# PacificBiosciences/minorseq

Hardware: NVIDIA B200
Metric: aligned CCS reads/sec pileup+call+phase (higher is better)
Workload: dtype u32 counts / f64 p-values

## Files before the change

### minorseq_b200/csrc/call.cu

```cuda
#include <algorithm>
#include <cstring>
#include <vector>
#include "fisher_core.h"
#include "handle.h"

namespace ms {

struct CallPos {
    int32_t gene, codon_index, col, ref_codon;
    uint32_t ntests;
};

struct CallConst {
    double P[4];
    double alpha, min_perc, max_perc;
};

__global__ void call_kernel(const uint32_t* __restrict__ codon, const CallPos* __restrict__ pos, int32_t npos,
                            CallConst cc, ms_variant* __restrict__ out, unsigned long long* __restrict__ nout,
                            unsigned long long cap) {
    const int warp = (blockIdx.x * blockDim.x + threadIdx.x) >> 5, lane = threadIdx.x & 31;
    if (warp >= npos) return;
    const CallPos ps = pos[warp];
    const uint32_t* h = codon + static_cast<size_t>(ps.col) * 64;
    const uint32_t k0 = h[lane], k1 = h[lane + 32];
    uint32_t n = k0 + k1;
#pragma unroll
    for (int o = 16; o > 0; o >>= 1) n += __shfl_xor_sync(0xffffffffu, n, o);
    if (n == 0) return;
    int ref = ps.ref_codon;
    if (ref < 0) {
        uint32_t bc = k0, bi = lane;
        if (k1 > bc) { bc = k1; bi = lane + 32; }
#pragma unroll
        for (int o = 16; o > 0; o >>= 1) {
            const uint32_t oc = __shfl_xor_sync(0xffffffffu, bc, o), oi = __shfl_xor_sync(0xffffffffu, bi, o);
            if (oc > bc || (oc == bc && oi < bi)) { bc = oc; bi = oi; }
        }
        ref = static_cast<int>(bi);
    }
#pragma unroll
    for (int half = 0; half < 2; ++half) {
        const int c = lane + 32 * half;
        const uint32_t k = half ? k1 : k0;
        if (c == ref || k == 0) continue;
        int nm = 0;
#pragma unroll
        for (int i = 0; i < 3; ++i) nm += (((ref >> (2 * i)) & 3) != ((c >> (2 * i)) & 3)) ? 1 : 0;
        const double ex = ceil(static_cast<double>(n) * cc.P[nm]);
        const uint32_t e = ex >= static_cast<double>(n) ? n : static_cast<uint32_t>(ex);
        if (k <= e && 0.5 * static_cast<double>(ps.ntests) >= cc.alpha) continue;
        const double p = fisher_greater(k, n - k, e, n - e, 1.000001 * cc.alpha / static_cast<double>(ps.ntests));
        if (!(p * static_cast<double>(ps.ntests) < cc.alpha)) continue;
        const double perc = 100.0 * static_cast<double>(k) / static_cast<double>(n);
        if (cc.min_perc >= 0.0 && !(perc > cc.min_perc)) continue;
        if (cc.max_perc >= 0.0 && !(perc < cc.max_perc)) continue;
        const unsigned long long slot = atomicAdd(nout, 1ULL);
        if (slot < cap) {
            ms_variant v;
            v.gene = ps.gene; v.codon_index = ps.codon_index; v.col = ps.col; v.ref_codon = ref; v.codon = c;
            v.count = k; v.coverage = n; v.expected = e; v.ntests = ps.ntests; v.pvalue = p;
            out[slot] = v;
        }
    }
}

static int base_code(char ch) {
    switch (ch) {
    case 'A': case 'a': return 0;
    case 'C': case 'c': return 1;
    case 'G': case 'g': return 2;
    case 'T': case 't': return 3;
    default: return -1;
    }
}

}

extern "C" {

void ms_call_params_default(ms_call_params* p) {
    if (!p) return;
    p->substitution_rate = 5e-4; p->deletion_rate = 3e-3; p->alpha = 0.01;
    p->min_perc = -1.0; p->max_perc = -1.0; p->region_begin = 0; p->region_end = 0;
}

// ... 52 lines not shown
    ms_variant* d_out = reinterpret_cast<ms_variant*>(base + 64);
    ms::CallPos* d_pos = reinterpret_cast<ms::CallPos*>(base + 64 + dev_cap * sizeof(ms_variant));
    constexpr size_t kQuick = 1024;
    const size_t stage_need = std::max(npos * sizeof(ms::CallPos), 64 + kQuick * sizeof(ms_variant));
    if (stage_need > h->call_stage_cap) {
        if (h->call_stage) cudaFreeHost(h->call_stage);
        h->call_stage = nullptr; h->call_stage_cap = 0;
        MS_CUDA(h, cudaMallocHost(&h->call_stage, stage_need + 4096));
        h->call_stage_cap = stage_need + 4096;
    }
    const size_t pos_bytes = npos * sizeof(ms::CallPos);
    const bool same_pos = h->call_pos_cache.size() == pos_bytes && memcmp(h->call_pos_cache.data(), pos.data(), pos_bytes) == 0;
    MS_CUDA(h, cudaMemsetAsync(d_n, 0, 8, h->stream));
    if (!same_pos) {
        memcpy(h->call_stage, pos.data(), pos_bytes);
        MS_CUDA(h, cudaMemcpyAsync(d_pos, h->call_stage, pos_bytes, cudaMemcpyHostToDevice, h->stream));
        MS_CUDA(h, cudaStreamSynchronize(h->stream));
        h->call_pos_cache.assign(reinterpret_cast<const uint8_t*>(pos.data()), reinterpret_cast<const uint8_t*>(pos.data()) + pos_bytes);
    }
    ms::CallConst cc;
    ms::codon_error_table(prm->substitution_rate, prm->deletion_rate, cc.P);
    cc.alpha = prm->alpha; cc.min_perc = prm->min_perc; cc.max_perc = prm->max_perc;
    const int threads = 128;
    const int blocks = static_cast<int>((npos * 32 + threads - 1) / threads);
    ms::call_kernel<<<blocks, threads, 0, h->stream>>>(h->d_counts + static_cast<size_t>(L) * 8, d_pos,
                                                       static_cast<int32_t>(npos), cc, d_out, d_n, dev_cap);
    h->launches++;
    MS_CUDA(h, cudaGetLastError());
    const size_t quick = std::min(kQuick, dev_cap);
    MS_CUDA(h, cudaMemcpyAsync(h->call_stage, base, 64 + quick * sizeof(ms_variant), cudaMemcpyDeviceToHost, h->stream));
    if (d_calls) *d_calls = d_out;
    if (d_ncalls) *d_ncalls = d_n;
    if (calls_cap) *calls_cap = static_cast<int64_t>(dev_cap);
    return MS_OK;
}

int ms_call_collect(ms_handle* h, bool synced, ms_variant* out, int64_t cap, int64_t* n) {
    if (!h || !n || (cap > 0 && !out)) return MS_ERR_ARG;
    *n = 0;
    if (h->call_npos == 0) return MS_OK;
    MS_CUDA(h, cudaSetDevice(h->device));
    if (!synced) MS_CUDA(h, cudaStreamSynchronize(h->stream));
    constexpr size_t kQuick = 1024;
    const size_t dev_cap = h->call_npos * 63;
    const size_t quick = std::min(kQuick, dev_cap);
    uint8_t* base = static_cast<uint8_t*>(h->d_call_buf);
    const ms_variant* d_out = reinterpret_cast<const ms_variant*>(base + 64);
// ... 31 lines not shown
```

### minorseq_b200/csrc/handle.h

```cpp
#pragma once
#include <cuda_runtime.h>
#include <stdint.h>
#include <string>
#include <vector>
#include "../../include/minorseq_b200.h"
#include <nvtx3/nvToolsExt.h>

struct MsRange {
    explicit MsRange(const char* name) { nvtxRangePushA(name); }
    ~MsRange() { nvtxRangePop(); }
    MsRange(const MsRange&) = delete;
    MsRange& operator=(const MsRange&) = delete;
};

struct DevBuf {
    void* p = nullptr;
    size_t cap = 0;
    cudaError_t ensure(size_t bytes) {
        if (bytes <= cap && p) return cudaSuccess;
        if (p) { cudaError_t e = cudaFree(p); p = nullptr; cap = 0; if (e != cudaSuccess) return e; }
        const size_t want = bytes + bytes / 4 + 256;
        cudaError_t e = cudaMalloc(&p, want);
        if (e == cudaSuccess) cap = want;
        return e;
// ... 44 lines not shown
    bool have_base = false;

    uint32_t* d_upload = nullptr;
    size_t upload_cap = 0;
    DevBuf b_rowstage[2];

    void* d_call_buf = nullptr;
    size_t call_cap = 0;
    void* call_stage = nullptr;
    size_t call_stage_cap = 0;
    std::vector<uint8_t> call_pos_cache;
    size_t call_npos = 0;

    int32_t V = 0, vwords = 0;
    int64_t phase_cap = 0, phase_n = 0;
    int32_t nblocklist = 0;
    int32_t phase_nrec = 0;
    bool phase_ordered = true;
    bool phase_partial_all = false;
    int64_t tab_size = 0, tab_size_max = 0, tab_hint = 0;
    int64_t gcap_hint = 0;
    bool table_valid = false;
    int table_attempt = 0;
    DevBuf b_plan;
    void* plan_stage = nullptr;
    uint32_t* counts_stage = nullptr; size_t counts_stage_words = 0;
    DevBuf b_var, b_blocklist, b_bits, b_flags, b_slot, b_tab_key, b_tab_cnt, b_tab_rep, b_ctr, b_groups, b_gather, b_rank, b_hap,
        b_pat, b_cooc, b_bits_t;
    DevBuf b_gslot, b_mt_key, b_mt_cnt, b_mt_rep, b_mslot, b_mindex, b_m_cnt, b_m_pat, b_m_rank, b_ord, b_keys, b_out, b_tc_tiles;
    DevBuf b_nw_seq, b_nw_hrow, b_nw_hcol, b_nw_dir;
    int32_t tc_tiles_V = -1;
    int cooc_variant = 0;
    bool linkage = false;
    bool link_ready = false;
    bool gram_valid = false;
    std::vector<int32_t> link_col;
    DevBuf b_mbits, b_link_gram, b_link_col, b_link_sig, b_link_rows, b_link_out;
    std::vector<uint32_t> groups_cnt, groups_pat;
    uint64_t groups_marg[4] = {0, 0, 0, 0};
    bool groups_valid = false;
    void* h_stage = nullptr;
    size_t h_stage_cap = 0;

    void* comm = nullptr;
    int world = 1, rank = 0;

// ... 21 lines not shown
```

### minorseq_b200/csrc/phase.cu

```cuda
#include <algorithm>
#include <cstring>
#include <numeric>
#include <vector>
#include "phase_internal.cuh"

namespace ms {

constexpr uint32_t kHdrFirst = 1u << 24, kHdrPacked = 1u << 25;

constexpr int kPhaseWarps = 8;
constexpr int kPhaseChunkMax = 16;

template <bool kClean>
__global__ void __launch_bounds__(kPhaseWarps * 32, 4) phase_bits_kernel(
    const uint4* __restrict__ packed, int64_t R, int32_t nblk, const int32_t* __restrict__ blocklist, int32_t NB, int32_t chunk, int32_t dbuf,
    const uint32_t* __restrict__ stream, int32_t nwords, int32_t vwords, int32_t ordered, int32_t partial_all,
    uint32_t* __restrict__ bits, uint8_t* __restrict__ flags, unsigned long long* __restrict__ ctr, const PhasePlan* __restrict__ plan,
    uint32_t* __restrict__ mbits) {
    extern __shared__ __align__(16) uint4 stage_sm[];
    if (plan) {
        if (plan->fallback) return;
        NB = plan->NB; nwords = plan->nwords; partial_all = plan->partial_all; ordered = 1;
    }
    const int warp = threadIdx.x >> 5, lane = threadIdx.x & 31;
    uint4* sm = stage_sm + static_cast<size_t>(warp) * (dbuf ? 2 : 1) * (chunk + 1) * 32 + lane;
    const int64_t nwarps = static_cast<int64_t>(gridDim.x) * kPhaseWarps;
    unsigned long long c_dam = 0, c_gap = 0, c_het = 0, c_par = 0;
    for (int64_t base = (static_cast<int64_t>(blockIdx.x) * kPhaseWarps + warp) * 32; base < R; base += nwarps * 32) {
        const int64_t r = base + lane;
        const bool live = r < R;
        const uint4* tile = packed + static_cast<size_t>(r >> 3) * nblk * 8;
        const uint32_t pos = static_cast<uint32_t>(r & 7);
        uint32_t fg = 0, fh = 0, fp = partial_all ? 1u : 0u;
        uint32_t word = 0, widx = 0xffffffffu;
        uint32_t mword = 0;
        uint32_t* myrow = bits + static_cast<size_t>(r) * vwords;
        uint32_t* mrow = kClean ? mbits + static_cast<size_t>(r) * vwords : nullptr;
        auto flush = [&]() {
            if (ordered) myrow[widx] = word;
            else if (word) myrow[widx] |= word;
            if constexpr (kClean) {
                if (ordered) mrow[widx] = mword;
                else if (mword) mrow[widx] |= mword;
            }
        };
// ... 89 lines not shown
                    if constexpr (kClean) mword |= __funnelshift_l(0u, __funnelshift_r(clean, 0u, w) & 1u, v);
                }
                p += nv;
            }
            __syncwarp();
            if (!dbuf && c0 + chunk < NB) stage_chunk(c0 + chunk, sm0);
        }
        if (live) {
            if (ordered && vwords == 1) {
                myrow[0] = word;
                if constexpr (kClean) mrow[0] = mword;
            } else if (widx != 0xffffffffu) {
                flush();
            }
            const uint32_t f = (fg ? MS_FLAG_GAP : 0) | (fh ? MS_FLAG_HET : 0) | (fp ? MS_FLAG_PARTIAL : 0);
            flags[r] = static_cast<uint8_t>(f);
            if (f) {
                ++c_dam;
                if (f & MS_FLAG_GAP) ++c_gap;
                if (f & MS_FLAG_HET) ++c_het;
                if (f & MS_FLAG_PARTIAL) ++c_par;
            }
        }
    }
#pragma unroll
    for (int o = 16; o > 0; o >>= 1) {
        c_dam += __shfl_xor_sync(0xffffffffu, c_dam, o);
        c_gap += __shfl_xor_sync(0xffffffffu, c_gap, o);
        c_het += __shfl_xor_sync(0xffffffffu, c_het, o);
        c_par += __shfl_xor_sync(0xffffffffu, c_par, o);
    }
    if (lane == 0 && c_dam) {
        atomicAdd(ctr + 0, c_dam);
        atomicAdd(ctr + 1, c_gap);
        atomicAdd(ctr + 2, c_het);
        atomicAdd(ctr + 3, c_par);
    }
}

constexpr int kPlanSlotWords = kPlanMaxLayers * 5 + kPlanMaxKeys;

__device__ __forceinline__ void rank_distinct(const int32_t* vals, int n, int lane, int32_t* first, int (&rank)[2]) {
    for (int e = 0; e < 2; ++e) {
        const int i = lane + 32 * e;
        int f = 0;
        if (i < n && vals[i] != 0x7fffffff) {
            f = 1;
            for (int j = 0; j < i; ++j) f &= vals[j] != vals[i];
        }
        first[i] = f;
    }
    __syncwarp();
    for (int e = 0; e < 2; ++e) {
        const int i = lane + 32 * e;
        int r = 0;
        if (i < n)
            for (int j = 0; j < n; ++j) r += (first[j] && vals[j] < vals[i]) ? 1 : 0;
        rank[e] = r;
    }
// ... 97 lines not shown
    }
    __syncwarp();
    if (s_fail) return;
    int total = 0;
    for (int e = 0; e < 2; ++e) {
        const int sl = lane + 32 * e;
        int off = 0;
        for (int t = 0; t < sl; ++t) off += s_nw[t];
        for (int k = 0; k < s_nw[sl]; ++k) stream[off + k] = s_words[sl][k];
        if (sl < NB) blocklist[sl] = s_blk[sl];
    }
    for (int t = 0; t < kPlanMaxBlocks; ++t) total += s_nw[t];
    if (lane < V) { plan->key_col[lane] = s_kc[lane]; plan->key_codon[lane] = s_kk[lane]; }
    __syncwarp();
    if (lane == 0) {
        plan->V = V; plan->NB = NB; plan->nwords = total; plan->partial_all = partial;
        __threadfence();
        plan->fallback = 0;
    }
}

__global__ void __launch_bounds__(256) phase_clear_kernel(unsigned long long* __restrict__ tab_key, uint32_t* __restrict__ tab_cnt,
                                                          long long* __restrict__ tab_rep, int64_t tab_size, unsigned long long* __restrict__ ctr,
                                                          unsigned long long last_resort) {
    const int64_t stride = static_cast<int64_t>(gridDim.x) * blockDim.x;
    for (int64_t i = static_cast<int64_t>(blockIdx.x) * blockDim.x + threadIdx.x; i < tab_size; i += stride) {
        tab_key[i] = 0ULL;
        tab_cnt[i] = 0u;
        tab_rep[i] = 0x7f7f7f7f7f7f7f7fLL;
    }
    if (blockIdx.x == 0 && threadIdx.x == 0) { ctr[4] = 0ULL; ctr[6] = 0ULL; ctr[7] = last_resort; }
}

__global__ void phase_insert_kernel(const uint32_t* __restrict__ bits, const uint8_t* __restrict__ flags, int64_t R,
                                    int32_t vwords, uint64_t seed, unsigned long long* tab_key, uint32_t* tab_cnt,
                                    long long* tab_rep, int64_t mask, int32_t* __restrict__ slot, unsigned long long* overflow) {
    const int64_t r = static_cast<int64_t>(blockIdx.x) * blockDim.x + threadIdx.x;
    const int lane = threadIdx.x & 31;
    const bool valid = r < R && flags[r] == 0;
    if (r < R && !valid) slot[r] = -1;
    if (__any_sync(0xffffffffu, *reinterpret_cast<volatile unsigned long long*>(overflow) != 0ULL)) {
        if (r < R) slot[r] = -1;
        return;
    }
    const uint32_t vmask = __ballot_sync(0xffffffffu, valid);
    if (!valid) return;
    const uint64_t key = pattern_hash(bits + static_cast<size_t>(r) * vwords, vwords, seed);
    const uint32_t peers = __match_any_sync(vmask, static_cast<unsigned long long>(key));
    const int leader = __ffs(peers) - 1;
    int64_t idx = -1;
    if (lane == leader) {
        int64_t probe = static_cast<int64_t>(key) & mask;
        for (int step = 0; step < 256; ++step) {
            const unsigned long long prev = atomicCAS(tab_key + probe, 0ULL, static_cast<unsigned long long>(key));
            if (prev == 0ULL || prev == key) { idx = probe; break; }
            probe = (probe + 1) & mask;
        }
        if (idx >= 0) {
            atomicAdd(tab_cnt + idx, static_cast<uint32_t>(__popc(peers)));
            atomicMin(tab_rep + idx, static_cast<long long>(r));
        } else {
            atomicAdd(overflow, 1ULL);
        }
    }
    idx = __shfl_sync(peers, idx, leader);
    slot[r] = static_cast<int32_t>(idx);
}

__global__ void phase_verify_kernel(const uint32_t* __restrict__ bits, int64_t R, int32_t vwords,
                                    const long long* __restrict__ tab_rep, const int32_t* __restrict__ slot,
                                    unsigned long long* collision) {
    const int64_t r = static_cast<int64_t>(blockIdx.x) * blockDim.x + threadIdx.x;
    if (r >= R || slot[r] < 0) return;
    const long long rep = tab_rep[slot[r]];
    if (rep == r) return;
    const uint32_t* a = bits + static_cast<size_t>(r) * vwords;
    const uint32_t* b = bits + static_cast<size_t>(rep) * vwords;
    for (int32_t i = 0; i < vwords; ++i)
        if (a[i] != b[i]) { atomicAdd(collision, 1ULL); return; }
}

__global__ void phase_compact_kernel(const uint32_t* __restrict__ tab_cnt, const long long* __restrict__ tab_rep,
                                     int64_t tab_size, const uint32_t* __restrict__ bits, int32_t vwords,
                                     unsigned long long* ngroups, uint32_t* __restrict__ g_cnt,
                                     uint32_t* __restrict__ g_pat, int32_t* __restrict__ g_slot, int64_t cap) {
    const int64_t i = static_cast<int64_t>(blockIdx.x) * blockDim.x + threadIdx.x;
    if (i >= tab_size || tab_cnt[i] == 0) return;
    const unsigned long long k = atomicAdd(ngroups, 1ULL);
    if (static_cast<int64_t>(k) < cap) {
        g_cnt[k] = tab_cnt[i];
        if (g_slot) g_slot[k] = static_cast<int32_t>(i);
        const uint32_t* src = bits + static_cast<size_t>(tab_rep[i]) * vwords;
        for (int32_t w = 0; w < vwords; ++w) g_pat[k * vwords + w] = src[w];
    }
}

__global__ void phase_rank_kernel(const uint32_t* __restrict__ ordered, int64_t H, int32_t vwords, uint64_t seed,
                                  const unsigned long long* __restrict__ tab_key, const long long* __restrict__ tab_rep,
                                  int64_t mask, const uint32_t* __restrict__ bits, int32_t* __restrict__ slot_rank) {
    const int64_t g = static_cast<int64_t>(blockIdx.x) * blockDim.x + threadIdx.x;
    if (g >= H) return;
    const uint32_t* pat = ordered + static_cast<size_t>(g) * vwords;
// ... 74 lines not shown

int ms_comm_allgather_bytes(ms_handle* h, const void* d_send, void* d_recv, size_t bytes_per_rank);
int ms_cooccurrence_tc_launch(ms_handle* h, const uint32_t* bt, int32_t V, int64_t rstride, int64_t R, int32_t* C);

namespace {

int phase_groups_copy_out(ms_handle* h, uint32_t* patterns, uint64_t* counts, int64_t cap, int64_t* H, ms_phase_counters* ctr);

constexpr int64_t kGroupCapInit = 4096;

}

namespace ms {

int phase_ensure_stage(ms_handle* h, size_t bytes) {
    if (bytes <= h->h_stage_cap) return MS_OK;
    if (h->h_stage) cudaFreeHost(h->h_stage);
    h->h_stage = nullptr; h->h_stage_cap = 0;
    MS_CUDA(h, cudaMallocHost(&h->h_stage, bytes + bytes / 4 + 4096));
    h->h_stage_cap = bytes + bytes / 4 + 4096;
    return MS_OK;
}

int phase_build_table(ms_handle* h, int attempt) {
    const int64_t R = h->phase_n;
    unsigned long long* ctr = phase_ctr(h);
    const unsigned long long last_resort = (h->tab_size >= h->tab_size_max || attempt >= 3) ? 1ULL : 0ULL;
    phase_clear_kernel<<<static_cast<int>(std::min<int64_t>((h->tab_size + 255) / 256, static_cast<int64_t>(h->num_sms) * 8)), 256, 0, h->stream>>>(
        h->b_tab_key.as<unsigned long long>(), h->b_tab_cnt.as<uint32_t>(), h->b_tab_rep.as<long long>(), h->tab_size, ctr, last_resort);
    h->launches++;
    if (R > 0) {
        const int grid = static_cast<int>((R + 255) / 256);
        phase_insert_kernel<<<grid, 256, 0, h->stream>>>(h->b_bits.as<uint32_t>(), h->b_flags.as<uint8_t>(), R, h->vwords,
                                                         phase_seed(attempt), h->b_tab_key.as<unsigned long long>(),
                                                         h->b_tab_cnt.as<uint32_t>(), h->b_tab_rep.as<long long>(),
                                                         h->tab_size - 1, h->b_slot.as<int32_t>(), ctr + 6);
        phase_verify_kernel<<<grid, 256, 0, h->stream>>>(h->b_bits.as<uint32_t>(), R, h->vwords, h->b_tab_rep.as<long long>(),
                                                         h->b_slot.as<int32_t>(), ctr + 4);
        h->launches += 2;
    }
    h->table_attempt = attempt;
    MS_CUDA(h, cudaGetLastError());
    return MS_OK;
}

int phase_compact(ms_handle* h, uint32_t* g_cnt, uint32_t* g_pat, int32_t* g_slot, int64_t cap) {
    MS_CUDA(h, cudaMemsetAsync(phase_ctr(h) + 5, 0, 8, h->stream));
    phase_compact_kernel<<<static_cast<int>((h->tab_size + 255) / 256), 256, 0, h->stream>>>(
        h->b_tab_cnt.as<uint32_t>(), h->b_tab_rep.as<long long>(), h->tab_size, h->b_bits.as<uint32_t>(), h->vwords, phase_ctr(h) + 5,
        g_cnt, g_pat, g_slot, cap);
    h->launches++;
    MS_CUDA(h, cudaGetLastError());
    return MS_OK;
}

int phase_grow_table(ms_handle* h) {
    if (h->tab_size >= h->tab_size_max) MS_FAIL(h, MS_ERR_CUDA, "haplotype table overflow at maximum size");
    h->tab_size = std::min<int64_t>(h->tab_size_max, h->tab_size * 8);
    h->tab_hint = h->tab_size;
    MS_CUDA(h, h->b_tab_key.ensure(static_cast<size_t>(h->tab_size) * 8));
    MS_CUDA(h, h->b_tab_cnt.ensure(static_cast<size_t>(h->tab_size) * 4));
    MS_CUDA(h, h->b_tab_rep.ensure(static_cast<size_t>(h->tab_size) * 8));
    h->table_valid = false;
    return MS_OK;
}
// ... 8 lines not shown
inline int build_table(ms_handle* h, int attempt) { return ms::phase_build_table(h, attempt); }

int phase_groups_copy_out(ms_handle* h, uint32_t* patterns, uint64_t* counts, int64_t cap, int64_t* H, ms_phase_counters* ctr) {
    const int32_t nw = h->vwords;
    const int64_t ng = static_cast<int64_t>(h->groups_cnt.size());
    const int64_t k = std::min<int64_t>(cap, ng);
    if (patterns && k > 0) memcpy(patterns, h->groups_pat.data(), static_cast<size_t>(k) * nw * 4);
    if (counts) for (int64_t i = 0; i < k; ++i) counts[i] = h->groups_cnt[i];
    *H = ng;
    if (ctr) {
        ctr->reported = 0; ctr->insufficient = 0;
        ctr->damaged = h->groups_marg[0]; ctr->gaps = h->groups_marg[1]; ctr->heteroduplex = h->groups_marg[2]; ctr->partial = h->groups_marg[3];
    }
    return MS_OK;
}

}

void ms_phase_set_smem_attr() {
    const int bytes = ms::kPhaseWarps * 2 * (ms::kPhaseChunkMax / 2 + 1) * 32 * static_cast<int>(sizeof(uint4)) >
                              ms::kPhaseWarps * (ms::kPhaseChunkMax + 1) * 32 * static_cast<int>(sizeof(uint4))
                          ? ms::kPhaseWarps * 2 * (ms::kPhaseChunkMax / 2 + 1) * 32 * static_cast<int>(sizeof(uint4))
                          : ms::kPhaseWarps * (ms::kPhaseChunkMax + 1) * 32 * static_cast<int>(sizeof(uint4));
    cudaFuncSetAttribute(ms::phase_bits_kernel<false>, cudaFuncAttributeMaxDynamicSharedMemorySize, bytes);
    cudaFuncSetAttribute(ms::phase_bits_kernel<true>, cudaFuncAttributeMaxDynamicSharedMemorySize, bytes);
}

extern "C" {

void ms_phase_free_internal(ms_handle* h) {
    DevBuf* all[] = {&h->b_plan, &h->b_var, &h->b_blocklist, &h->b_bits, &h->b_flags, &h->b_slot, &h->b_tab_key, &h->b_tab_cnt, &h->b_tab_rep,
                     &h->b_ctr, &h->b_groups, &h->b_gather, &h->b_rank, &h->b_hap, &h->b_pat, &h->b_cooc, &h->b_bits_t,
                     &h->b_gslot, &h->b_mt_key, &h->b_mt_cnt, &h->b_mt_rep, &h->b_mslot, &h->b_mindex, &h->b_m_cnt, &h->b_m_pat, &h->b_m_rank,
                     &h->b_ord, &h->b_keys, &h->b_out, &h->b_tc_tiles,
                     &h->b_nw_seq, &h->b_nw_hrow, &h->b_nw_hcol, &h->b_nw_dir,
                     &h->b_mbits, &h->b_link_gram, &h->b_link_col, &h->b_link_sig, &h->b_link_rows, &h->b_link_out};
    for (DevBuf* b : all) b->release();
    if (h->h_stage) cudaFreeHost(h->h_stage);
    h->h_stage = nullptr; h->h_stage_cap = 0;
    if (h->plan_stage) cudaFreeHost(h->plan_stage);
    h->plan_stage = nullptr;
    h->phase_cap = h->phase_n = 0; h->V = 0; h->vwords = 0; h->table_valid = false;
    h->link_ready = h->gram_valid = false;
}

int ms_phase_begin(ms_handle* h, const int32_t* var_col, const int32_t* var_codon, int32_t V, int64_t max_reads) {
    if (!h || h->L <= 0 || V < 0 || max_reads < 0 || (V > 0 && (!var_col || !var_codon))) return MS_ERR_ARG;
    MS_CUDA(h, cudaSetDevice(h->device));
// ... 144 lines not shown
    MS_CUDA(h, cudaSetDevice(h->device));
    h->table_valid = false;
    h->groups_valid = false;
    h->gram_valid = false;
    uint32_t* bits = h->b_bits.as<uint32_t>() + static_cast<size_t>(h->phase_n) * h->vwords;
    uint32_t* mbits = h->link_ready ? h->b_mbits.as<uint32_t>() + static_cast<size_t>(h->phase_n) * h->vwords : nullptr;
    uint8_t* flags = h->b_flags.as<uint8_t>() + h->phase_n;
    const uint4* pk = reinterpret_cast<const uint4*>(d_packed);
    const uint32_t* stream = h->b_var.as<uint32_t>();
    unsigned long long* ctr = ctr_ptr(h);
    if (!(h->phase_ordered && h->vwords == 1)) {
        MS_CUDA(h, cudaMemsetAsync(bits, 0, static_cast<size_t>(R) * h->vwords * 4, h->stream));
        if (mbits) MS_CUDA(h, cudaMemsetAsync(mbits, 0, static_cast<size_t>(R) * h->vwords * 4, h->stream));
    }
    MS_STAGE_BEGIN(h, MS_STAGE_PHASE_BITS);
    {
        const bool dbuf = h->nblocklist > ms::kPhaseChunkMax;
        const int chunk = dbuf ? ms::kPhaseChunkMax / 2 : std::min(ms::kPhaseChunkMax, h->nblocklist);
        const size_t smem = static_cast<size_t>(ms::kPhaseWarps) * (dbuf ? 2 : 1) * (chunk + 1) * 32 * sizeof(uint4);
        const int per_sm = std::max(1, std::min(6, static_cast<int>((h->max_smem + 1024) / (smem + 1024))));
        const int64_t want = (R + ms::kPhaseWarps * 32 - 1) / (ms::kPhaseWarps * 32);
        const int grid = static_cast<int>(std::max<int64_t>(1, std::min<int64_t>(want, static_cast<int64_t>(h->num_sms) * per_sm)));
        if (mbits)
            ms::phase_bits_kernel<true><<<grid, ms::kPhaseWarps * 32, smem, h->stream>>>(pk, R, h->nblk, h->b_blocklist.as<int32_t>(), h->nblocklist, chunk,
                                                                                        dbuf ? 1 : 0, stream, h->phase_nrec, h->vwords,
                                                                                        h->phase_ordered ? 1 : 0, h->phase_partial_all ? 1 : 0, bits, flags,
                                                                                        ctr, nullptr, mbits);
        else
            ms::phase_bits_kernel<false><<<grid, ms::kPhaseWarps * 32, smem, h->stream>>>(pk, R, h->nblk, h->b_blocklist.as<int32_t>(), h->nblocklist, chunk, dbuf ? 1 : 0,
                                                                                         stream, h->phase_nrec, h->vwords, h->phase_ordered ? 1 : 0,
                                                                                         h->phase_partial_all ? 1 : 0, bits, flags, ctr, nullptr, nullptr);
    }
    MS_STAGE_END(h, MS_STAGE_PHASE_BITS);
    h->launches++;
    MS_CUDA(h, cudaGetLastError());
    h->phase_n += R;
    return MS_OK;
}

}

int ms_phase_planned_dev(ms_handle* h, const ms_variant* d_calls, const unsigned long long* d_ncalls, int64_t calls_cap,
                         const uint32_t* d_packed, int64_t R, ms::PhasePlan** d_plan_out) {
    if (!h || h->L <= 0 || R < 0 || !d_calls || !d_ncalls || (R > 0 && !d_packed)) return MS_ERR_ARG;
    MS_CUDA(h, cudaSetDevice(h->device));
    h->V = 0;
    h->vwords = 1;
    h->link_ready = h->gram_valid = false;
    h->phase_cap = std::max<int64_t>(1, R);
    h->phase_n = 0;
    h->table_valid = false;
    h->groups_valid = false;
    int64_t ts_max = 1024;
    while (ts_max < 2 * h->phase_cap) ts_max <<= 1;
    h->tab_size_max = ts_max;
    const int64_t ts = std::min<int64_t>(ts_max, std::max<int64_t>(1 << 16, h->tab_hint));
    h->tab_size = ts;
    const size_t plan_bytes = sizeof(ms::PhasePlan);
    const bool grow = static_cast<size_t>(ms::kPlanStreamWords) * 4 > h->b_var.cap || static_cast<size_t>(ms::kPlanMaxBlocks) * 4 > h->b_blocklist.cap ||
                      static_cast<size_t>(h->phase_cap) * 4 > h->b_bits.cap || static_cast<size_t>(h->phase_cap) > h->b_flags.cap ||
                      static_cast<size_t>(ts) * 8 > h->b_tab_key.cap || !h->b_ctr.p || plan_bytes > h->b_plan.cap;
    if (grow) MS_CUDA(h, cudaStreamSynchronize(h->stream));
    MS_CUDA(h, h->b_var.ensure(static_cast<size_t>(ms::kPlanStreamWords) * 4));
    MS_CUDA(h, h->b_blocklist.ensure(static_cast<size_t>(ms::kPlanMaxBlocks) * 4));
    MS_CUDA(h, h->b_bits.ensure(static_cast<size_t>(h->phase_cap) * 4));
    MS_CUDA(h, h->b_flags.ensure(static_cast<size_t>(h->phase_cap)));
    MS_CUDA(h, h->b_slot.ensure(static_cast<size_t>(h->phase_cap) * 4));
    MS_CUDA(h, h->b_tab_key.ensure(static_cast<size_t>(ts) * 8));
    MS_CUDA(h, h->b_tab_cnt.ensure(static_cast<size_t>(ts) * 4));
    MS_CUDA(h, h->b_tab_rep.ensure(static_cast<size_t>(ts) * 8));
    MS_CUDA(h, h->b_ctr.ensure(64));
    MS_CUDA(h, h->b_plan.ensure(plan_bytes));
    int rc = ensure_stage(h, 1 << 20);
    if (rc != MS_OK) return rc;
    ms::PhasePlan* d_plan = h->b_plan.as<ms::PhasePlan>();
    MS_CUDA(h, cudaMemsetAsync(h->b_ctr.p, 0, 64, h->stream));
    ms::phase_plan_kernel<<<1, 32, 0, h->stream>>>(d_calls, d_ncalls, calls_cap, h->L, d_plan, h->b_blocklist.as<int32_t>(), h->b_var.as<uint32_t>());
    h->launches++;
    if (R > 0) {
        MS_STAGE_BEGIN(h, MS_STAGE_PHASE_BITS);
        const int chunk = ms::kPhaseChunkMax;
        const size_t smem = static_cast<size_t>(ms::kPhaseWarps) * (chunk + 1) * 32 * sizeof(uint4);
        const int per_sm = std::max(1, std::min(6, static_cast<int>((h->max_smem + 1024) / (smem + 1024))));
        const int64_t want = (R + ms::kPhaseWarps * 32 - 1) / (ms::kPhaseWarps * 32);
        const int grid = static_cast<int>(std::max<int64_t>(1, std::min<int64_t>(want, static_cast<int64_t>(h->num_sms) * per_sm)));
        ms::phase_bits_kernel<false><<<grid, ms::kPhaseWarps * 32, smem, h->stream>>>(reinterpret_cast<const uint4*>(d_packed), R, h->nblk,
                                                                                     h->b_blocklist.as<int32_t>(), 0, chunk, 0, h->b_var.as<uint32_t>(), 0, 1,
                                                                                     1, 0, h->b_bits.as<uint32_t>(), h->b_flags.as<uint8_t>(), ctr_ptr(h),
                                                                                     d_plan, nullptr);
        MS_STAGE_END(h, MS_STAGE_PHASE_BITS);
        h->launches++;
    }
    MS_CUDA(h, cudaGetLastError());
    h->phase_n = R;
    if (d_plan_out) *d_plan_out = d_plan;
    return MS_OK;
}

void ms_phase_planned_adopt(ms_handle* h, int32_t V) { h->V = V; }

int ms_gram_dev(ms_handle* h, const uint32_t* const* mats, int nmat, int32_t dim, int32_t* G) {
    const int32_t V = h->V, nw = h->vwords;
    const int64_t R = h->phase_n;
    const bool tensor = h->cooc_variant == 2 || (h->cooc_variant == 0 && V >= 256 && R >= 32768);
    const int64_t rwords = tensor ? 4 * ((R + 127) / 128) : std::max<int64_t>(1, (R + 31) / 32);
    const size_t gbytes = std::max<size_t>(4, static_cast<size_t>(dim) * dim * 4);
    const size_t mat_words = static_cast<size_t>(nw) * 32 * rwords;
    MS_CUDA(h, h->b_bits_t.ensure(std::max<size_t>(16, nmat * mat_words * 4)));
    MS_CUDA(h, cudaMemsetAsync(G, 0, gbytes, h->stream));
    if (V > 0 && rwords > 0) {
        const int64_t nwarps = rwords * nw;
        for (int k = 0; k < nmat; ++k) {
            ms::bits_transpose_kernel<<<static_cast<unsigned>((nwarps * 32 + 255) / 256), 256, 0, h->stream>>>(mats[k], R, nw, rwords,
                                                                                                             h->b_bits_t.as<uint32_t>() + k * mat_words);
            h->launches++;
        }
        MS_STAGE_BEGIN(h, MS_STAGE_COOCCURRENCE);
// ... 158 lines not shown

int ms_phase_assign(ms_handle* h, const uint32_t* ordered_patterns, int64_t H, int32_t* hap_id) {
    if (!h || !h->b_bits.p || H < 0 || (H > 0 && !ordered_patterns) || !hap_id) return MS_ERR_ARG;
    MS_CUDA(h, cudaSetDevice(h->device));
    if (!h->table_valid) {
        if (h->comm) MS_FAIL(h, MS_ERR_ARG, "ms_phase_assign: call ms_phase_groups (on every rank) first");
        int64_t dummy = 0;
        int rc = ms_phase_groups(h, nullptr, nullptr, 0, &dummy, nullptr);
        if (rc != MS_OK) return rc;
    }
    const int64_t R = h->phase_n;
    const int32_t nw = h->vwords;
    MS_CUDA(h, h->b_rank.ensure(static_cast<size_t>(h->tab_size) * 4));
    MS_CUDA(h, h->b_hap.ensure(static_cast<size_t>(std::max<int64_t>(1, R)) * 4));
    MS_CUDA(h, h->b_pat.ensure(static_cast<size_t>(std::max<int64_t>(1, H)) * nw * 4));
    MS_CUDA(h, cudaMemsetAsync(h->b_rank.p, 0xff, static_cast<size_t>(h->tab_size) * 4, h->stream));
    if (H > 0) {
        MS_CUDA(h, cudaMemcpyAsync(h->b_pat.p, ordered_patterns, static_cast<size_t>(H) * nw * 4, cudaMemcpyHostToDevice, h->stream));
        ms::phase_rank_kernel<<<static_cast<int>((H + 127) / 128), 128, 0, h->stream>>>(
            h->b_pat.as<uint32_t>(), H, nw, phase_seed(h->table_attempt), h->b_tab_key.as<unsigned long long>(),
            h->b_tab_rep.as<long long>(), h->tab_size - 1, h->b_bits.as<uint32_t>(), h->b_rank.as<int32_t>());
        h->launches++;
    }
    if (R > 0) {
        ms::phase_assign_kernel<<<static_cast<int>((R + 255) / 256), 256, 0, h->stream>>>(h->b_slot.as<int32_t>(), h->b_rank.as<int32_t>(), R,
                                                                                         h->b_hap.as<int32_t>());
        h->launches++;
        MS_CUDA(h, cudaMemcpyAsync(hap_id, h->b_hap.p, static_cast<size_t>(R) * 4, cudaMemcpyDeviceToHost, h->stream));
    }
    MS_CUDA(h, cudaStreamSynchronize(h->stream));
    MS_CUDA(h, cudaGetLastError());
    return MS_OK;
}

int ms_phase_device(ms_handle* h, uint32_t** d_bits, uint8_t** d_flags, int64_t* R) {
    if (!h || !h->b_bits.p) return MS_ERR_ARG;
    if (d_bits) *d_bits = h->b_bits.as<uint32_t>();
    if (d_flags) *d_flags = h->b_flags.as<uint8_t>();
    if (R) *R = h->phase_n;
    return MS_OK;
}

int ms_set_cooccurrence_variant(ms_handle* h, int32_t variant) {
    if (!h || variant < 0 || variant > 2) return MS_ERR_ARG;
    h->cooc_variant = variant;
    return MS_OK;
// ... 18 lines not shown
```

### minorseq_b200/csrc/phase_internal.cuh

```cuda
#pragma once
#include "handle.h"

namespace ms {

__device__ __forceinline__ uint64_t mix64d(uint64_t x) {
    x ^= x >> 30; x *= 0xbf58476d1ce4e5b9ULL;
    x ^= x >> 27; x *= 0x94d049bb133111ebULL;
    x ^= x >> 31;
    return x;
}

__device__ __forceinline__ uint64_t pattern_hash(const uint32_t* w, int32_t vwords, uint64_t seed) {
    uint64_t hsh = seed;
    for (int32_t i = 0; i < vwords; ++i) hsh = mix64d(hsh ^ (static_cast<uint64_t>(w[i]) + 0x9E3779B97F4A7C15ULL * (i + 1)));
    return hsh ? hsh : 1ULL;
}

__host__ __device__ __forceinline__ bool pattern_less(const uint32_t* a, const uint32_t* b, int32_t nw) {
    for (int32_t i = 0; i < nw; ++i)
        if (a[i] != b[i]) return a[i] < b[i];
    return false;
}

inline uint64_t phase_seed(int attempt) { return 0x6d696e6f72736571ULL + 0x9E3779B97F4A7C15ULL * static_cast<uint64_t>(attempt); }

inline unsigned long long* phase_ctr(ms_handle* h) { return h->b_ctr.as<unsigned long long>(); }

constexpr int kPlanMaxKeys = 32, kPlanMaxCalls = 64, kPlanMaxBlocks = 64, kPlanMaxLayers = 4;
constexpr int kPlanStreamWords = kPlanMaxBlocks * kPlanMaxLayers * 5 + kPlanMaxKeys;
struct PhasePlan {
    int32_t V, NB, nwords, partial_all, fallback, ncalls;
    int32_t key_col[kPlanMaxKeys], key_codon[kPlanMaxKeys];
};

int phase_ensure_stage(ms_handle* h, size_t bytes);
int phase_build_table(ms_handle* h, int attempt);
int phase_compact(ms_handle* h, uint32_t* g_cnt, uint32_t* g_pat, int32_t* g_slot, int64_t cap);
int phase_grow_table(ms_handle* h);

}
```

### minorseq_b200/csrc/phase_order.cu

```cuda
#include <algorithm>
#include <cstring>
#include "phase_internal.cuh"

int ms_comm_allgather_bytes(ms_handle* h, const void* d_send, void* d_recv, size_t bytes_per_rank);

namespace ms {

constexpr int64_t kSmallSort = 4096;
constexpr uint32_t kSentinel = 0xffffffffu;
constexpr int kLocalSpan = 2048;

struct OrderOut {
    unsigned long long* res;
    uint32_t* rank;
    uint32_t* o_cnt;
    uint32_t* o_pat;
    int64_t ocap;
    uint32_t min_reads;
};

__device__ __forceinline__ unsigned long long warp_sum64(unsigned long long v) {
#pragma unroll
    for (int o = 16; o > 0; o >>= 1) v += __shfl_xor_sync(0xffffffffu, v, o);
    return v;
// ... 392 lines not shown
            MS_CUDA(h, cudaStreamSynchronize(h->stream));
            memcpy(res, st, 64);
        }
        *H = M;
        if (nreported) *nreported = static_cast<int64_t>(res[1]);
        if (ctr) {
            ctr->reported = res[2]; ctr->insufficient = res[3];
            ctr->damaged = marg[0]; ctr->gaps = marg[1]; ctr->heteroduplex = marg[2]; ctr->partial = marg[3];
        }
        break;
    }
    const int64_t need = std::min<int64_t>(ocap, M);
    uint8_t* st = static_cast<uint8_t*>(h->h_stage);
    const uint8_t* outb = h->b_out.as<uint8_t>();
    bool pending = false;
    if (need > 0 && off_pat + static_cast<size_t>(need) * nw * 4 > first_copy) {
        if (off_cnt + static_cast<size_t>(need) * 4 > first_copy)
            MS_CUDA(h, cudaMemcpyAsync(st + off_cnt, outb + off_cnt, static_cast<size_t>(need) * 4, cudaMemcpyDeviceToHost, h->stream));
        MS_CUDA(h, cudaMemcpyAsync(st + off_pat, outb + off_pat, static_cast<size_t>(need) * nw * 4, cudaMemcpyDeviceToHost, h->stream));
        pending = true;
    }
    if (hap_id && h->phase_n > 0) {
        MS_CUDA(h, h->b_hap.ensure(static_cast<size_t>(h->phase_n) * 4));
        ms::hap_assign_kernel<<<grid_for(h->phase_n, 256), 256, 0, h->stream>>>(h->b_slot.as<int32_t>(), h->b_rank.as<int32_t>(), h->phase_n,
                                                                               h->b_hap.as<int32_t>());
        h->launches++;
        MS_CUDA(h, cudaMemcpyAsync(hap_id, h->b_hap.p, static_cast<size_t>(h->phase_n) * 4, cudaMemcpyDeviceToHost, h->stream));
        pending = true;
    }
    if (pending) MS_CUDA(h, cudaStreamSynchronize(h->stream));
    MS_CUDA(h, cudaGetLastError());
    if (need > 0) {
        memcpy(patterns, st + off_pat, static_cast<size_t>(need) * nw * 4);
        const uint32_t* c = reinterpret_cast<const uint32_t*>(st + off_cnt);
        for (int64_t i = 0; i < need; ++i) counts[i] = c[i];
    }
    return MS_OK;
}
```

Baseline: 1.539 billion.

## Fuse haplotype grouping into phase bits kernel and defer per-read slot lookup

The planned phase-bits kernel now groups identical single-word patterns in a shared-memory hash table per CTA using warp match, then flushes the group counts into the global hash table. This removes the separate insert pass and the per-read slot writes on the fast path. Slots are rebuilt lazily by a read-only probe kernel only when haplotype IDs are requested, and the verify pass is skipped when patterns fit in one word. The call kernel also splits each position across two warps, one per codon half. The fused kernel uses more shared memory per CTA, which may reduce occupancy, and shared atomics can contend on skewed data.

```diff
diff --git a/minorseq_b200/csrc/call.cu b/minorseq_b200/csrc/call.cu
--- a/minorseq_b200/csrc/call.cu
+++ b/minorseq_b200/csrc/call.cu
@@ -19,7 +19,8 @@
 __global__ void call_kernel(const uint32_t* __restrict__ codon, const CallPos* __restrict__ pos, int32_t npos,
                             CallConst cc, ms_variant* __restrict__ out, unsigned long long* __restrict__ nout,
                             unsigned long long cap) {
-    const int warp = (blockIdx.x * blockDim.x + threadIdx.x) >> 5, lane = threadIdx.x & 31;
+    const int gw = (blockIdx.x * blockDim.x + threadIdx.x) >> 5, lane = threadIdx.x & 31;
+    const int warp = gw >> 1, half = gw & 1;
     if (warp >= npos) return;
     const CallPos ps = pos[warp];
     const uint32_t* h = codon + static_cast<size_t>(ps.col) * 64;
@@ -39,29 +40,26 @@
         }
         ref = static_cast<int>(bi);
     }
+    const int c = lane + 32 * half;
+    const uint32_t k = half ? k1 : k0;
+    if (c == ref || k == 0) return;
+    int nm = 0;
 #pragma unroll
-    for (int half = 0; half < 2; ++half) {
-        const int c = lane + 32 * half;
-        const uint32_t k = half ? k1 : k0;
-        if (c == ref || k == 0) continue;
-        int nm = 0;
-#pragma unroll
-        for (int i = 0; i < 3; ++i) nm += (((ref >> (2 * i)) & 3) != ((c >> (2 * i)) & 3)) ? 1 : 0;
-        const double ex = ceil(static_cast<double>(n) * cc.P[nm]);
-        const uint32_t e = ex >= static_cast<double>(n) ? n : static_cast<uint32_t>(ex);
-        if (k <= e && 0.5 * static_cast<double>(ps.ntests) >= cc.alpha) continue;
-        const double p = fisher_greater(k, n - k, e, n - e, 1.000001 * cc.alpha / static_cast<double>(ps.ntests));
-        if (!(p * static_cast<double>(ps.ntests) < cc.alpha)) continue;
-        const double perc = 100.0 * static_cast<double>(k) / static_cast<double>(n);
-        if (cc.min_perc >= 0.0 && !(perc > cc.min_perc)) continue;
-        if (cc.max_perc >= 0.0 && !(perc < cc.max_perc)) continue;
-        const unsigned long long slot = atomicAdd(nout, 1ULL);
-        if (slot < cap) {
-            ms_variant v;
-            v.gene = ps.gene; v.codon_index = ps.codon_index; v.col = ps.col; v.ref_codon = ref; v.codon = c;
-            v.count = k; v.coverage = n; v.expected = e; v.ntests = ps.ntests; v.pvalue = p;
-            out[slot] = v;
-        }
+    for (int i = 0; i < 3; ++i) nm += (((ref >> (2 * i)) & 3) != ((c >> (2 * i)) & 3)) ? 1 : 0;
+    const double ex = ceil(static_cast<double>(n) * cc.P[nm]);
+    const uint32_t e = ex >= static_cast<double>(n) ? n : static_cast<uint32_t>(ex);
+    if (k <= e && 0.5 * static_cast<double>(ps.ntests) >= cc.alpha) return;
+    const double p = fisher_greater(k, n - k, e, n - e, 1.000001 * cc.alpha / static_cast<double>(ps.ntests));
+    if (!(p * static_cast<double>(ps.ntests) < cc.alpha)) return;
+    const double perc = 100.0 * static_cast<double>(k) / static_cast<double>(n);
+    if (cc.min_perc >= 0.0 && !(perc > cc.min_perc)) return;
+    if (cc.max_perc >= 0.0 && !(perc < cc.max_perc)) return;
+    const unsigned long long slot = atomicAdd(nout, 1ULL);
+    if (slot < cap) {
+        ms_variant v;
+        v.gene = ps.gene; v.codon_index = ps.codon_index; v.col = ps.col; v.ref_codon = ref; v.codon = c;
+        v.count = k; v.coverage = n; v.expected = e; v.ntests = ps.ntests; v.pvalue = p;
+        out[slot] = v;
     }
 }
 
@@ -160,7 +158,7 @@
     ms::codon_error_table(prm->substitution_rate, prm->deletion_rate, cc.P);
     cc.alpha = prm->alpha; cc.min_perc = prm->min_perc; cc.max_perc = prm->max_perc;
     const int threads = 128;
-    const int blocks = static_cast<int>((npos * 32 + threads - 1) / threads);
+    const int blocks = static_cast<int>((npos * 64 + threads - 1) / threads);
     ms::call_kernel<<<blocks, threads, 0, h->stream>>>(h->d_counts + static_cast<size_t>(L) * 8, d_pos,
                                                        static_cast<int32_t>(npos), cc, d_out, d_n, dev_cap);
     h->launches++;
diff --git a/minorseq_b200/csrc/handle.h b/minorseq_b200/csrc/handle.h
--- a/minorseq_b200/csrc/handle.h
+++ b/minorseq_b200/csrc/handle.h
@@ -90,6 +90,7 @@
     int64_t gcap_hint = 0;
     bool table_valid = false;
     int table_attempt = 0;
+    bool slot_valid = false;
     DevBuf b_plan;
     void* plan_stage = nullptr;
     uint32_t* counts_stage = nullptr; size_t counts_stage_words = 0;
diff --git a/minorseq_b200/csrc/phase.cu b/minorseq_b200/csrc/phase.cu
--- a/minorseq_b200/csrc/phase.cu
+++ b/minorseq_b200/csrc/phase.cu
@@ -11,16 +11,73 @@
 constexpr int kPhaseWarps = 8;
 constexpr int kPhaseChunkMax = 16;
 
-template <bool kClean>
+struct GroupTable {
+    unsigned long long* key;
+    uint32_t* cnt;
+    long long* rep;
+    int64_t mask;
+    uint64_t seed;
+    unsigned long long* overflow;
+};
+
+__device__ __forceinline__ int64_t group_table_add(const GroupTable& g, uint64_t key, uint32_t n, long long rep) {
+    int64_t probe = static_cast<int64_t>(key) & g.mask, idx = -1;
+    for (int step = 0; step < 256; ++step) {
+        const unsigned long long prev = atomicCAS(g.key + probe, 0ULL, static_cast<unsigned long long>(key));
+        if (prev == 0ULL || prev == key) { idx = probe; break; }
+        probe = (probe + 1) & g.mask;
+    }
+    if (idx >= 0) {
+        atomicAdd(g.cnt + idx, n);
+        atomicMin(g.rep + idx, rep);
+    } else {
+        atomicAdd(g.overflow, 1ULL);
+    }
+    return idx;
+}
+
+constexpr int kCtaGroupsLog2 = 8, kCtaGroups = 1 << kCtaGroupsLog2, kCtaProbe = 32;
+struct CtaGroups {
+    unsigned long long key[kCtaGroups];
+    long long rep[kCtaGroups];
+    uint32_t cnt[kCtaGroups];
+};
+
+__device__ __forceinline__ void cta_group_add(CtaGroups* t, const GroupTable& g, uint32_t word, uint32_t n, long long rep) {
+    const unsigned long long k = (1ULL << 32) | word;
+    uint32_t i = (word * 0x9E3779B1u) >> (32 - kCtaGroupsLog2);
+    for (int step = 0; step < kCtaProbe; ++step) {
+        const unsigned long long prev = atomicCAS(t->key + i, 0ULL, k);
+        if (prev == 0ULL || prev == k) {
+            atomicAdd(t->cnt + i, n);
+            atomicMin(t->rep + i, rep);
+            return;
+        }
+        i = (i + 1) & (kCtaGroups - 1);
+    }
+    group_table_add(g, pattern_hash(&word, 1, g.seed), n, rep);
+}
+
+template <bool kClean, bool kGroup>
 __global__ void __launch_bounds__(kPhaseWarps * 32, 4) phase_bits_kernel(
     const uint4* __restrict__ packed, int64_t R, int32_t nblk, const int32_t* __restrict__ blocklist, int32_t NB, int32_t chunk, int32_t dbuf,
     const uint32_t* __restrict__ stream, int32_t nwords, int32_t vwords, int32_t ordered, int32_t partial_all,
     uint32_t* __restrict__ bits, uint8_t* __restrict__ flags, unsigned long long* __restrict__ ctr, const PhasePlan* __restrict__ plan,
-    uint32_t* __restrict__ mbits) {
+    uint32_t* __restrict__ mbits, GroupTable gtab) {
     extern __shared__ __align__(16) uint4 stage_sm[];
     if (plan) {
         if (plan->fallback) return;
         NB = plan->NB; nwords = plan->nwords; partial_all = plan->partial_all; ordered = 1;
+    }
+    CtaGroups* cta = nullptr;
+    if constexpr (kGroup) {
+        cta = reinterpret_cast<CtaGroups*>(stage_sm + static_cast<size_t>(kPhaseWarps) * (dbuf ? 2 : 1) * (chunk + 1) * 32);
+        for (int i = threadIdx.x; i < kCtaGroups; i += blockDim.x) {
+            cta->key[i] = 0ULL;
+            cta->cnt[i] = 0u;
+            cta->rep[i] = 0x7f7f7f7f7f7f7f7fLL;
+        }
+        __syncthreads();
     }
     const int warp = threadIdx.x >> 5, lane = threadIdx.x & 31;
     uint4* sm = stage_sm + static_cast<size_t>(warp) * (dbuf ? 2 : 1) * (chunk + 1) * 32 + lane;
@@ -156,6 +213,14 @@
                 if (f & MS_FLAG_PARTIAL) ++c_par;
             }
         }
+        if constexpr (kGroup) {
+            const bool grp = live && (fg | fh | fp) == 0u;
+            const uint32_t gmask = __ballot_sync(0xffffffffu, grp);
+            if (grp) {
+                const uint32_t peers = __match_any_sync(gmask, word);
+                if (lane == __ffs(peers) - 1) cta_group_add(cta, gtab, word, static_cast<uint32_t>(__popc(peers)), static_cast<long long>(r));
+            }
+        }
     }
 #pragma unroll
     for (int o = 16; o > 0; o >>= 1) {
@@ -169,6 +234,16 @@
         atomicAdd(ctr + 1, c_gap);
         atomicAdd(ctr + 2, c_het);
         atomicAdd(ctr + 3, c_par);
+    }
+    if constexpr (kGroup) {
+        __syncthreads();
+        for (int i = threadIdx.x; i < kCtaGroups; i += blockDim.x) {
+            const unsigned long long k = cta->key[i];
+            if (k) {
+                const uint32_t w = static_cast<uint32_t>(k);
+                group_table_add(gtab, pattern_hash(&w, 1, gtab.seed), cta->cnt[i], cta->rep[i]);
+            }
+        }
     }
 }
 
@@ -312,47 +387,36 @@
 
 __global__ void __launch_bounds__(256) phase_clear_kernel(unsigned long long* __restrict__ tab_key, uint32_t* __restrict__ tab_cnt,
                                                           long long* __restrict__ tab_rep, int64_t tab_size, unsigned long long* __restrict__ ctr,
-                                                          unsigned long long last_resort) {
+                                                          unsigned long long last_resort, int32_t all) {
     const int64_t stride = static_cast<int64_t>(gridDim.x) * blockDim.x;
     for (int64_t i = static_cast<int64_t>(blockIdx.x) * blockDim.x + threadIdx.x; i < tab_size; i += stride) {
         tab_key[i] = 0ULL;
         tab_cnt[i] = 0u;
         tab_rep[i] = 0x7f7f7f7f7f7f7f7fLL;
     }
-    if (blockIdx.x == 0 && threadIdx.x == 0) { ctr[4] = 0ULL; ctr[6] = 0ULL; ctr[7] = last_resort; }
+    if (blockIdx.x == 0 && threadIdx.x < 8) {
+        if (threadIdx.x == 7) ctr[7] = last_resort;
+        else if (all || threadIdx.x == 4 || threadIdx.x == 6) ctr[threadIdx.x] = 0ULL;
+    }
 }
 
 __global__ void phase_insert_kernel(const uint32_t* __restrict__ bits, const uint8_t* __restrict__ flags, int64_t R,
-                                    int32_t vwords, uint64_t seed, unsigned long long* tab_key, uint32_t* tab_cnt,
-                                    long long* tab_rep, int64_t mask, int32_t* __restrict__ slot, unsigned long long* overflow) {
+                                    int32_t vwords, GroupTable g, int32_t* __restrict__ slot) {
     const int64_t r = static_cast<int64_t>(blockIdx.x) * blockDim.x + threadIdx.x;
     const int lane = threadIdx.x & 31;
     const bool valid = r < R && flags[r] == 0;
     if (r < R && !valid) slot[r] = -1;
-    if (__any_sync(0xffffffffu, *reinterpret_cast<volatile unsigned long long*>(overflow) != 0ULL)) {
+    if (__any_sync(0xffffffffu, *reinterpret_cast<volatile unsigned long long*>(g.overflow) != 0ULL)) {
         if (r < R) slot[r] = -1;
         return;
     }
     const uint32_t vmask = __ballot_sync(0xffffffffu, valid);
     if (!valid) return;
-    const uint64_t key = pattern_hash(bits + static_cast<size_t>(r) * vwords, vwords, seed);
+    const uint64_t key = pattern_hash(bits + static_cast<size_t>(r) * vwords, vwords, g.seed);
     const uint32_t peers = __match_any_sync(vmask, static_cast<unsigned long long>(key));
     const int leader = __ffs(peers) - 1;
     int64_t idx = -1;
-    if (lane == leader) {
-        int64_t probe = static_cast<int64_t>(key) & mask;
-        for (int step = 0; step < 256; ++step) {
-            const unsigned long long prev = atomicCAS(tab_key + probe, 0ULL, static_cast<unsigned long long>(key));
-            if (prev == 0ULL || prev == key) { idx = probe; break; }
-            probe = (probe + 1) & mask;
-        }
-        if (idx >= 0) {
-            atomicAdd(tab_cnt + idx, static_cast<uint32_t>(__popc(peers)));
-            atomicMin(tab_rep + idx, static_cast<long long>(r));
-        } else {
-            atomicAdd(overflow, 1ULL);
-        }
-    }
+    if (lane == leader) idx = group_table_add(g, key, static_cast<uint32_t>(__popc(peers)), static_cast<long long>(r));
     idx = __shfl_sync(peers, idx, leader);
     slot[r] = static_cast<int32_t>(idx);
 }
@@ -368,6 +432,24 @@
     const uint32_t* b = bits + static_cast<size_t>(rep) * vwords;
     for (int32_t i = 0; i < vwords; ++i)
         if (a[i] != b[i]) { atomicAdd(collision, 1ULL); return; }
+}
+
+__global__ void phase_slot_kernel(const uint32_t* __restrict__ bits, const uint8_t* __restrict__ flags, int64_t R, int32_t vwords,
+                                  uint64_t seed, const unsigned long long* __restrict__ tab_key, int64_t mask, int32_t* __restrict__ slot) {
+    const int64_t r = static_cast<int64_t>(blockIdx.x) * blockDim.x + threadIdx.x;
+    if (r >= R) return;
+    int64_t idx = -1;
+    if (flags[r] == 0) {
+        const uint64_t key = pattern_hash(bits + static_cast<size_t>(r) * vwords, vwords, seed);
+        int64_t probe = static_cast<int64_t>(key) & mask;
+        for (int64_t step = 0; step <= mask; ++step) {
+            const unsigned long long k = tab_key[probe];
+            if (k == key) { idx = probe; break; }
+            if (k == 0ULL) break;
+            probe = (probe + 1) & mask;
+        }
+    }
+    slot[r] = static_cast<int32_t>(idx);
 }
 
 __global__ void phase_compact_kernel(const uint32_t* __restrict__ tab_cnt, const long long* __restrict__ tab_rep,
@@ -488,25 +570,50 @@
     return MS_OK;
 }
 
+static GroupTable group_table(ms_handle* h, int attempt) {
+    return GroupTable{h->b_tab_key.as<unsigned long long>(), h->b_tab_cnt.as<uint32_t>(), h->b_tab_rep.as<long long>(), h->tab_size - 1,
+                      phase_seed(attempt), phase_ctr(h) + 6};
+}
+
+static void clear_table(ms_handle* h, int attempt, bool all) {
+    const unsigned long long last_resort = (h->tab_size >= h->tab_size_max || attempt >= 3) ? 1ULL : 0ULL;
+    phase_clear_kernel<<<static_cast<int>(std::min<int64_t>((h->tab_size + 255) / 256, static_cast<int64_t>(h->num_sms) * 8)), 256, 0, h->stream>>>(
+        h->b_tab_key.as<unsigned long long>(), h->b_tab_cnt.as<uint32_t>(), h->b_tab_rep.as<long long>(), h->tab_size, phase_ctr(h), last_resort,
+        all ? 1 : 0);
+    h->launches++;
+}
+
 int phase_build_table(ms_handle* h, int attempt) {
     const int64_t R = h->phase_n;
-    unsigned long long* ctr = phase_ctr(h);
-    const unsigned long long last_resort = (h->tab_size >= h->tab_size_max || attempt >= 3) ? 1ULL : 0ULL;
-    phase_clear_kernel<<<static_cast<int>(std::min<int64_t>((h->tab_size + 255) / 256, static_cast<int64_t>(h->num_sms) * 8)), 256, 0, h->stream>>>(
-        h->b_tab_key.as<unsigned long long>(), h->b_tab_cnt.as<uint32_t>(), h->b_tab_rep.as<long long>(), h->tab_size, ctr, last_resort);
-    h->launches++;
+    clear_table(h, attempt, false);
     if (R > 0) {
         const int grid = static_cast<int>((R + 255) / 256);
         phase_insert_kernel<<<grid, 256, 0, h->stream>>>(h->b_bits.as<uint32_t>(), h->b_flags.as<uint8_t>(), R, h->vwords,
-                                                         phase_seed(attempt), h->b_tab_key.as<unsigned long long>(),
-                                                         h->b_tab_cnt.as<uint32_t>(), h->b_tab_rep.as<long long>(),
-                                                         h->tab_size - 1, h->b_slot.as<int32_t>(), ctr + 6);
-        phase_verify_kernel<<<grid, 256, 0, h->stream>>>(h->b_bits.as<uint32_t>(), R, h->vwords, h->b_tab_rep.as<long long>(),
-                                                         h->b_slot.as<int32_t>(), ctr + 4);
-        h->launches += 2;
+                                                         group_table(h, attempt), h->b_slot.as<int32_t>());
+        h->launches++;
+        if (h->vwords > 1) {
+            phase_verify_kernel<<<grid, 256, 0, h->stream>>>(h->b_bits.as<uint32_t>(), R, h->vwords, h->b_tab_rep.as<long long>(),
+                                                             h->b_slot.as<int32_t>(), phase_ctr(h) + 4);
+            h->launches++;
+        }
     }
     h->table_attempt = attempt;
+    h->slot_valid = true;
     MS_CUDA(h, cudaGetLastError());
+    return MS_OK;
+}
+
+int phase_ensure_slots(ms_handle* h) {
+    if (h->slot_valid) return MS_OK;
+    const int64_t R = h->phase_n;
+    if (R > 0) {
+        phase_slot_kernel<<<static_cast<int>((R + 255) / 256), 256, 0, h->stream>>>(h->b_bits.as<uint32_t>(), h->b_flags.as<uint8_t>(), R, h->vwords,
+                                                                                    phase_seed(h->table_attempt), h->b_tab_key.as<unsigned long long>(),
+                                                                                    h->tab_size - 1, h->b_slot.as<int32_t>());
+        h->launches++;
+        MS_CUDA(h, cudaGetLastError());
+    }
+    h->slot_valid = true;
     return MS_OK;
 }
 
@@ -561,8 +668,10 @@
                               ms::kPhaseWarps * (ms::kPhaseChunkMax + 1) * 32 * static_cast<int>(sizeof(uint4))
                           ? ms::kPhaseWarps * 2 * (ms::kPhaseChunkMax / 2 + 1) * 32 * static_cast<int>(sizeof(uint4))
                           : ms::kPhaseWarps * (ms::kPhaseChunkMax + 1) * 32 * static_cast<int>(sizeof(uint4));
-    cudaFuncSetAttribute(ms::phase_bits_kernel<false>, cudaFuncAttributeMaxDynamicSharedMemorySize, bytes);
-    cudaFuncSetAttribute(ms::phase_bits_kernel<true>, cudaFuncAttributeMaxDynamicSharedMemorySize, bytes);
+    cudaFuncSetAttribute(ms::phase_bits_kernel<false, false>, cudaFuncAttributeMaxDynamicSharedMemorySize, bytes);
+    cudaFuncSetAttribute(ms::phase_bits_kernel<true, false>, cudaFuncAttributeMaxDynamicSharedMemorySize, bytes);
+    cudaFuncSetAttribute(ms::phase_bits_kernel<false, true>, cudaFuncAttributeMaxDynamicSharedMemorySize,
+                         ms::kPhaseWarps * (ms::kPhaseChunkMax + 1) * 32 * static_cast<int>(sizeof(uint4)) + static_cast<int>(sizeof(ms::CtaGroups)));
 }
 
 extern "C" {
@@ -753,14 +862,15 @@
         const int64_t want = (R + ms::kPhaseWarps * 32 - 1) / (ms::kPhaseWarps * 32);
         const int grid = static_cast<int>(std::max<int64_t>(1, std::min<int64_t>(want, static_cast<int64_t>(h->num_sms) * per_sm)));
         if (mbits)
-            ms::phase_bits_kernel<true><<<grid, ms::kPhaseWarps * 32, smem, h->stream>>>(pk, R, h->nblk, h->b_blocklist.as<int32_t>(), h->nblocklist, chunk,
-                                                                                        dbuf ? 1 : 0, stream, h->phase_nrec, h->vwords,
-                                                                                        h->phase_ordered ? 1 : 0, h->phase_partial_all ? 1 : 0, bits, flags,
-                                                                                        ctr, nullptr, mbits);
+            ms::phase_bits_kernel<true, false><<<grid, ms::kPhaseWarps * 32, smem, h->stream>>>(pk, R, h->nblk, h->b_blocklist.as<int32_t>(), h->nblocklist, chunk,
+                                                                                               dbuf ? 1 : 0, stream, h->phase_nrec, h->vwords,
+                                                                                               h->phase_ordered ? 1 : 0, h->phase_partial_all ? 1 : 0, bits, flags,
+                                                                                               ctr, nullptr, mbits, ms::GroupTable{});
         else
-            ms::phase_bits_kernel<false><<<grid, ms::kPhaseWarps * 32, smem, h->stream>>>(pk, R, h->nblk, h->b_blocklist.as<int32_t>(), h->nblocklist, chunk, dbuf ? 1 : 0,
-                                                                                         stream, h->phase_nrec, h->vwords, h->phase_ordered ? 1 : 0,
-                                                                                         h->phase_partial_all ? 1 : 0, bits, flags, ctr, nullptr, nullptr);
+            ms::phase_bits_kernel<false, false><<<grid, ms::kPhaseWarps * 32, smem, h->stream>>>(pk, R, h->nblk, h->b_blocklist.as<int32_t>(), h->nblocklist, chunk,
+                                                                                                dbuf ? 1 : 0, stream, h->phase_nrec, h->vwords, h->phase_ordered ? 1 : 0,
+                                                                                                h->phase_partial_all ? 1 : 0, bits, flags, ctr, nullptr, nullptr,
+                                                                                                ms::GroupTable{});
     }
     MS_STAGE_END(h, MS_STAGE_PHASE_BITS);
     h->launches++;
@@ -805,25 +915,28 @@
     int rc = ensure_stage(h, 1 << 20);
     if (rc != MS_OK) return rc;
     ms::PhasePlan* d_plan = h->b_plan.as<ms::PhasePlan>();
-    MS_CUDA(h, cudaMemsetAsync(h->b_ctr.p, 0, 64, h->stream));
+    ms::clear_table(h, 0, true);
     ms::phase_plan_kernel<<<1, 32, 0, h->stream>>>(d_calls, d_ncalls, calls_cap, h->L, d_plan, h->b_blocklist.as<int32_t>(), h->b_var.as<uint32_t>());
     h->launches++;
     if (R > 0) {
         MS_STAGE_BEGIN(h, MS_STAGE_PHASE_BITS);
         const int chunk = ms::kPhaseChunkMax;
-        const size_t smem = static_cast<size_t>(ms::kPhaseWarps) * (chunk + 1) * 32 * sizeof(uint4);
+        const size_t smem = static_cast<size_t>(ms::kPhaseWarps) * (chunk + 1) * 32 * sizeof(uint4) + sizeof(ms::CtaGroups);
         const int per_sm = std::max(1, std::min(6, static_cast<int>((h->max_smem + 1024) / (smem + 1024))));
         const int64_t want = (R + ms::kPhaseWarps * 32 - 1) / (ms::kPhaseWarps * 32);
         const int grid = static_cast<int>(std::max<int64_t>(1, std::min<int64_t>(want, static_cast<int64_t>(h->num_sms) * per_sm)));
-        ms::phase_bits_kernel<false><<<grid, ms::kPhaseWarps * 32, smem, h->stream>>>(reinterpret_cast<const uint4*>(d_packed), R, h->nblk,
-                                                                                     h->b_blocklist.as<int32_t>(), 0, chunk, 0, h->b_var.as<uint32_t>(), 0, 1,
-                                                                                     1, 0, h->b_bits.as<uint32_t>(), h->b_flags.as<uint8_t>(), ctr_ptr(h),
-                                                                                     d_plan, nullptr);
+        ms::phase_bits_kernel<false, true><<<grid, ms::kPhaseWarps * 32, smem, h->stream>>>(reinterpret_cast<const uint4*>(d_packed), R, h->nblk,
+                                                                                           h->b_blocklist.as<int32_t>(), 0, chunk, 0, h->b_var.as<uint32_t>(), 0, 1,
+                                                                                           1, 0, h->b_bits.as<uint32_t>(), h->b_flags.as<uint8_t>(), ctr_ptr(h),
+                                                                                           d_plan, nullptr, ms::group_table(h, 0));
         MS_STAGE_END(h, MS_STAGE_PHASE_BITS);
         h->launches++;
     }
     MS_CUDA(h, cudaGetLastError());
     h->phase_n = R;
+    h->table_valid = true;
+    h->table_attempt = 0;
+    h->slot_valid = false;
     if (d_plan_out) *d_plan_out = d_plan;
     return MS_OK;
 }
@@ -1028,6 +1141,8 @@
             h->b_tab_rep.as<long long>(), h->tab_size - 1, h->b_bits.as<uint32_t>(), h->b_rank.as<int32_t>());
         h->launches++;
     }
+    int rc = ms::phase_ensure_slots(h);
+    if (rc != MS_OK) return rc;
     if (R > 0) {
         ms::phase_assign_kernel<<<static_cast<int>((R + 255) / 256), 256, 0, h->stream>>>(h->b_slot.as<int32_t>(), h->b_rank.as<int32_t>(), R,
                                                                                          h->b_hap.as<int32_t>());
diff --git a/minorseq_b200/csrc/phase_internal.cuh b/minorseq_b200/csrc/phase_internal.cuh
--- a/minorseq_b200/csrc/phase_internal.cuh
+++ b/minorseq_b200/csrc/phase_internal.cuh
@@ -35,6 +35,7 @@
 
 int phase_ensure_stage(ms_handle* h, size_t bytes);
 int phase_build_table(ms_handle* h, int attempt);
+int phase_ensure_slots(ms_handle* h);
 int phase_compact(ms_handle* h, uint32_t* g_cnt, uint32_t* g_pat, int32_t* g_slot, int64_t cap);
 int phase_grow_table(ms_handle* h);
 
diff --git a/minorseq_b200/csrc/phase_order.cu b/minorseq_b200/csrc/phase_order.cu
--- a/minorseq_b200/csrc/phase_order.cu
+++ b/minorseq_b200/csrc/phase_order.cu
@@ -438,6 +438,8 @@
     }
     if (hap_id && h->phase_n > 0) {
         MS_CUDA(h, h->b_hap.ensure(static_cast<size_t>(h->phase_n) * 4));
+        int rc = ms::phase_ensure_slots(h);
+        if (rc != MS_OK) return rc;
         ms::hap_assign_kernel<<<grid_for(h->phase_n, 256), 256, 0, h->stream>>>(h->b_slot.as<int32_t>(), h->b_rank.as<int32_t>(), h->phase_n,
                                                                                h->b_hap.as<int32_t>());
         h->launches++;
```

Result: faster. 1.647 billion (median of 6 runs) (+7.0%).
